# rishabhgoel0213/ZeroClone

Hardware: AMD Instinct MI355X
Metric: MCTS node-expansions/sec (whole node), Connect4 800 sims/move at 1/2/4/8 MI355X (higher is better)
Workload: dtype f64

## Files before the change

zeroclone_amd/csrc/c4_search.hip:

```cpp
#include "c4_device.h"
#include "counter_rng.h"

namespace zc {
namespace {


__device__ __forceinline__ uint64_t readlane64(uint64_t x, int l) {
    return ((uint64_t)(uint32_t)__builtin_amdgcn_readlane((int)(x >> 32), l) << 32) |
           (uint64_t)(uint32_t)__builtin_amdgcn_readlane((int)x, l);
}

__device__ __forceinline__ uint32_t mbcnt(uint64_t m) {
    return __builtin_amdgcn_mbcnt_hi((uint32_t)(m >> 32), __builtin_amdgcn_mbcnt_lo((uint32_t)m, 0u));
}

__device__ __forceinline__ uint32_t scan_add32(uint32_t x) {
    x += (uint32_t)__builtin_amdgcn_update_dpp(0, (int)x, 0x111, 0xF, 0xF, false);
    x += (uint32_t)__builtin_amdgcn_update_dpp(0, (int)x, 0x112, 0xF, 0xF, false);
    x += (uint32_t)__builtin_amdgcn_update_dpp(0, (int)x, 0x114, 0xF, 0xF, false);
    x += (uint32_t)__builtin_amdgcn_update_dpp(0, (int)x, 0x118, 0xF, 0xF, false);
    x += (uint32_t)__builtin_amdgcn_update_dpp(0, (int)x, 0x142, 0xA, 0xF, false);
    x += (uint32_t)__builtin_amdgcn_update_dpp(0, (int)x, 0x143, 0xC, 0xF, false);
    return x;
}
// ... 4 lines not shown
    x |= (uint32_t)__builtin_amdgcn_update_dpp(0, (int)x, 0x112, 0xF, 0xF, false);
    y |= (uint32_t)__builtin_amdgcn_update_dpp(0, (int)y, 0x112, 0xF, 0xF, false);
    x |= (uint32_t)__builtin_amdgcn_update_dpp(0, (int)x, 0x114, 0xF, 0xF, false);
    y |= (uint32_t)__builtin_amdgcn_update_dpp(0, (int)y, 0x114, 0xF, 0xF, false);
    x |= (uint32_t)__builtin_amdgcn_update_dpp(0, (int)x, 0x118, 0xF, 0xF, false);
    y |= (uint32_t)__builtin_amdgcn_update_dpp(0, (int)y, 0x118, 0xF, 0xF, false);
}

__device__ __forceinline__ uint64_t in_vgpr(uint64_t x) {
    __asm__("" : "+v"(x));
    return x;
}
__device__ __forceinline__ int neg_if_le(uint32_t a, uint32_t b, int y) {
    int r;
    __asm__("s_cmp_le_u32 %1, %2\n\ts_cselect_b32 %0, -1, %3" : "=s"(r) : "s"(a), "s"(b), "s"(y) : "scc");
    return r;
}
extern "C" __device__ int zc_writelane(int x, int l, int old) __asm("llvm.amdgcn.writelane.i32");
__device__ __forceinline__ uint32_t ff1(uint64_t m) {
    uint32_t r;
    __asm__("s_ff1_i32_b64 %0, %1" : "=s"(r) : "s"(m));
    return r;
}

#ifndef ZC_RV
#define ZC_RV 0
#endif
__device__ __forceinline__ void set_prio(int lvl) {
    if (lvl >= 3) __builtin_amdgcn_s_setprio(3);
    else if (lvl == 2) __builtin_amdgcn_s_setprio(2);
    else if (lvl == 1) __builtin_amdgcn_s_setprio(1);
    else __builtin_amdgcn_s_setprio(0);
}
#if defined(ZC_DIAG_WASTE) || defined(ZC_DIAG_UCT)
#define ZC_ROLLOUT_COUNTS 0
#else
#define ZC_ROLLOUT_COUNTS 1
#endif
#ifndef ZC_RSTAMP
#define ZC_RSTAMP 0
#endif
#define RMARK(k)                                                    \
    do {                                                            \
        if (ZC_RSTAMP && sub) {                                     \
            __builtin_amdgcn_sched_barrier(0);                      \
            const uint64_t now_ = __builtin_amdgcn_s_memtime();     \
            __builtin_amdgcn_sched_barrier(0);                      \
            if (ZC_RSTAMP == (k)) *sub += now_ - t_;                \
            t_ = now_;                                              \
        }                                                           \
    } while (0)
template <class R>
__device__ void c4_rollouts(Leaf *L, int nb, R &rng, const uint32_t *s_order, Counters &cn,
                            uint64_t *sub = nullptr) {
    uint64_t t_ = ZC_RSTAMP && sub ? __builtin_amdgcn_s_memtime() : 0;
    const uint32_t lane = lane_id();
    const uint32_t lrow = lane >> 4;
    constexpr uint32_t kTop3 = ViewBits<R>::kBits - 3u;
    const uint32_t *const s_dorder = draw_order_table(s_order);
    const uint64_t second_rows = __ballot((lrow & 1u) != 0);
    const uint32_t d1 = lrow < 2 ? 1u : 6u, d2 = lrow < 2 ? 7u : 8u;
    const uint32_t pairbits = lane < 49u ? (1u << (lane / 7u)) | (1u << (lane % 7u)) : 0u;
    __builtin_amdgcn_s_waitcnt(0x0F70);
    for (int g = 0; g < nb; g += 64) {
      uint32_t lm_v = 0, ow_v = 0, hp_v = 0;
      int room_v = 0;
      int val_v = 0, q_v = 0;
      {
        const int jj = g + (int)lane;
        if (jj < nb) {
            lm_v = L[jj].meta;
            ow_v = s_dorder[lm_v >> 25];
            const uint64_t x0 = L[jj].p0, x1 = L[jj].p1;
            const uint64_t op_v = (lm_v >> 24) & 1u ? x0 : x1;
            room_v = has_four(op_v) ? -2 : 41 - __popcll(x0 | x1);
            const uint64_t oc = x0 | x1;
            for (int c = 0; c < 7; ++c) hp_v |= (uint32_t)__popcll((oc >> (7 * c)) & 0x3Full) << (4 * c);
#if ZC_ROLLOUT_COUNTS
            cn.blocks += room_v >= 0 ? 1 : 0;
#endif
        }
      }
      const int jend = min(nb, g + 64);
      for (int j = g; j < jend; ++j) {
        RMARK(6);
        const int jl = j - g;
        const uint32_t lm = (uint32_t)__builtin_amdgcn_readlane((int)lm_v, jl);
        uint4 pw;
        __builtin_memcpy(&pw, &L[j], sizeof pw);
        uint64_t x0 = ((uint64_t)pw.y << 32) | pw.x, x1 = ((uint64_t)pw.w << 32) | pw.z;
        uint64_t S1 = (lm >> 24) & 1u ? ~second_rows : second_rows;
        uint32_t hp = (uint32_t)__builtin_amdgcn_readlane((int)hp_v, jl);
        const uint32_t low0 = (uint32_t)__builtin_amdgcn_readlane((int)ow_v, jl);
        const int room0 = __builtin_amdgcn_readlane(room_v, jl);
        int val = (room0 + 1) >> 1;
        int q = 0;
        RMARK(1);
        if (room0 >= 0) {
            int room = room0;
            int mask = (int)(lm >> 25);
            uint32_t ow = low0;
            uint32_t thr = (ow >> 24) & 15u;
            uint32_t owp = s_dorder[(uint32_t)mask & ~pairbits];
            uint32_t ew, l0, lf, endlane, endply, col, sc;
            uint64_t F, mine;
            auto block = [&]() __attribute__((always_inline)) {
                RMARK(6);
                uint32_t wv;
                uint64_t A;
                rng_need(rng);
                wv = rng_view(rng) >> kTop3;
                A = __ballot(wv < thr);
                if (__builtin_expect(A == 0ull, 0)) {
                    do {
                        rng_eat(rng, (uint32_t)kWin);
                        rng_need(rng);
                        wv = rng_view(rng) >> kTop3;
                        A = __ballot(wv < thr);
                    } while (A == 0ull);
                }
                RMARK(2);
                const uint32_t cap_r = min((uint32_t)room, 30u);
                uint32_t qk = mbcnt(A);
                col = (ow >> (3 * wv)) & 7u;
                uint32_t one = mask_sel0(A, 1u << (4 * col));
                sc = scan_add32(one);
                uint32_t row = ((sc - one + hp) >> (4 * col)) & 15u;
                uint32_t nacc = (uint32_t)__popcll(A);
                F = __ballot(row == 5u);
                uint64_t E0 = A & (F | __ballot(qk >= min(cap_r, nacc - 1u)));
                l0 = (uint32_t)__builtin_ctzll(E0);
                const uint64_t G = A & F & __ballot(qk < cap_r);
                lf = ff1(G);
#ifdef ZC_DIAG_WASTE
                const uint32_t l0f = l0;
#endif
                RMARK(3);
                if (lf == l0) {
                    const uint32_t cf = (uint32_t)__builtin_amdgcn_readlane((int)col, (int)lf);
                    const uint32_t ow2 = (uint32_t)__builtin_amdgcn_readlane((int)owp, (int)(8u * cf));
                    const uint32_t thr2 = (ow2 >> 24) & 15u;
                    const uint64_t high = ~1ull << lf;
                    A = (A & ~high) | (__ballot(wv < thr2) & high);
                    qk = mbcnt(A);
                    col = mask_sel(high, col, (ow2 >> (3 * wv)) & 7u);
                    one = mask_sel0(A, 1u << (4 * col));
                    sc = scan_add32(one);
                    row = ((sc - one + hp) >> (4 * col)) & 15u;
                    nacc = (uint32_t)__popcll(A);
                    F = __ballot(row == 5u) & high;
                    E0 = A & (F | __ballot(qk >= min(cap_r, nacc - 1u)));
                    l0 = (uint32_t)__builtin_ctzll(E0);
                }
                RMARK(4);
                const uint32_t c = ((qk & 1u) << 4) | ((qk >> 1) & 15u) | (qk & 32u);
                const uint32_t b = __umul24(col, 7u) + row;
                const uint32_t pl = (uint32_t)__builtin_amdgcn_ds_permute((int)(mask_sel(A, 63u, c) << 2), (int)b);
                const uint32_t pb = __builtin_amdgcn_permlane32_swap(pl, pl, false, false)[0];
                const uint64_t bit = 1ull << (pb & 63u);
                uint32_t blo = (uint32_t)bit, bhi = (uint32_t)(bit >> 32);
                scan_or16x2(blo, bhi);
                mine = ((uint64_t)bhi << 32) | blo;
                x0 = in_vgpr(x0);
                x1 = in_vgpr(x1);
                const uint64_t bd = (((uint64_t)mask_sel(S1, (uint32_t)(x0 >> 32), (uint32_t)(x1 >> 32)) << 32) |
                                     mask_sel(S1, (uint32_t)x0, (uint32_t)x1)) | mine;
                const uint64_t m1 = bd & (bd >> d1), m2 = bd & (bd >> d2);
                const uint64_t f4 = (m1 & (m1 >> (2 * d1))) | (m2 & (m2 >> (2 * d2)));
                const uint64_t W = __ballot(f4 != 0ull);
                const uint32_t W32 = (uint32_t)W | (uint32_t)(W >> 32);
                const uint64_t Ew = A & __ballot(((W32 >> (c & 31u)) & 1u) != 0u);
                ew = ff1(Ew);
                endlane = min(ew, l0);
                endply = (uint32_t)__builtin_amdgcn_readlane((int)qk, (int)endlane);
                rng_eat(rng, endlane + 1u);
#ifdef ZC_DIAG_WASTE
                cn.add(cn.blocks, lf == l0f && endlane < lf ? 1 : 0);
                cn.add(cn.plies, lf == l0f ? 1 : 0);
#endif
                room -= (int)endply + 1;
                RMARK(5);
// ... 68 lines not shown
                    const uint32_t h = (uint32_t)__popcll(((me | op) >> (7u * col)) & 0x3Full);
                    me |= 1ull << (7u * col + h);
                    ++q;
                    ++stones;
                    if (h == 5u) legal &= ~(1u << col);
                    if (has_four(me)) {
                        val = (q & 1) ? 1 : -1;
                        break;
                    }
                    if (stones == 42) {
                        val = 0;
                        break;
                    }
                    const uint64_t t = me;
                    me = op;
                    op = t;
                }
            }
            L[j].val = val;
        }
        int tot = q;
        for (int o = 32; o > 0; o >>= 1) tot += __shfl_xor(tot, o);
        cn.add(cn.plies, tot);
    }
}


__constant__ const uint64_t kEvery[8] = {0ull,
                                         0xFFFFFFFFFFFFFFFFull,
                                         0x5555555555555555ull,
                                         0x9249249249249249ull,
                                         0x1111111111111111ull,
                                         0x1084210842108421ull,
                                         0x1041041041041041ull,
                                         0x8102040810204081ull};

__device__ __forceinline__ uint64_t lanes_in(int lo, int hi) {
    const uint64_t below_hi = hi >= 64 ? ~0ull : (1ull << hi) - 1ull;
    return below_hi & ~((1ull << lo) - 1ull);
}


__device__ __forceinline__ float max8(float v) {
    float m;
    __asm__("s_nop 1\n\t"
            "v_max_f32_dpp %0, %1, %1 quad_perm:[1,0,3,2] row_mask:0xf bank_mask:0xf\n\t"
            "s_nop 1\n\t"
            "v_max_f32_dpp %0, %0, %0 quad_perm:[2,3,0,1] row_mask:0xf bank_mask:0xf\n\t"
            "s_nop 1\n\t"
            "v_max_f32_dpp %0, %0, %0 row_half_mirror row_mask:0xf bank_mask:0xf"
            : "=&v"(m)
            : "v"(v));
    return m;
}
__device__ __forceinline__ int uct_select8(uint64_t vmask, int32_t na, int32_t wa, double lg, double c, float cf,
                                           float delta, int *how = nullptr) {
    const float r = __builtin_amdgcn_rcpf((float)na);
    const float s = __builtin_amdgcn_sqrtf((float)lg * r);
    const float S = __builtin_fmaf(cf, s, (float)wa * r);
    const float Sv = __uint_as_float(mask_sel(vmask, 0xFF800000u, __float_as_uint(S)));
    const float thr = max8(Sv) - delta;
    const uint64_t C = vmask & ~__ballot(Sv < thr);
    const int first = __builtin_ctzll(C);
    if (how) *how = 0;
    if ((C & (C - 1ull)) == 0ull) return first;
    const int32_t na0 = __builtin_amdgcn_readlane(na, first), wa0 = __builtin_amdgcn_readlane(wa, first);
    if (how) *how = 1;
    if ((C & ~__ballot(((na ^ na0) | (wa ^ wa0)) == 0)) == 0ull) return first;
    if (how) *how = 2;
    const bool valid = (vmask >> (lane_id() & 7u)) & 1ull;
    const double q = valid ? (double)wa / (double)na : 0.0;
    const double v = valid ? fma(c, sqrt(lg / (double)na), q) : -INFINITY;
    int bi;
    max8_first(v, &bi);
    return bi;
}

__device__ __forceinline__ WalkEnd walk_hbm_prefetch(const Tree &t, ConstDouble *logtab, uint64_t rp0, uint64_t rp1,
                                                     int rturn, int done, double c, float delta, Counters &cn,
                                                     int &status) {
    const uint32_t lane = lane_id();
    const uint32_t k = lane & 7u, cs = lane >> 3;
    const float cf = (float)c;
    (void)cn;
    int node = 0, depth = 0, turn = rturn, nN = done;
    uint64_t b0 = rp0, b1 = rp1;
    uint32_t pathv = (lane == 0) ? 0x00FF0000u : 0u;
    const uint8_t *R0 = t.rec(0);
    uint32_t u = uni(((const uint32_t *)R0)[1]), ow = uni(((const uint32_t *)R0)[3]);
    uint32_t ch = ((const uint16_t *)(R0 + 16))[k];
    int32_t na = ((const int32_t *)(R0 + 32))[k];
    int32_t wa = ((const int32_t *)(R0 + 64))[k];
    for (;;) {
        if (untried_count(u)) break;
        if (depth >= kMaxDepth - 2) {
            status = ZC_STATUS_INTERNAL;
            u = 0;
            break;
        }
        const uint32_t nm = u >> 28;
        const uint32_t cid = (uint32_t)__builtin_amdgcn_ds_bpermute((int)(cs << 2), (int)ch);
        uint32_t pch = 0xFFFFu, phd = 0u;
        int32_t pna = 0, pwa = 0;
        if (cs < nm && cid != 0xFFFFu) {
            const uint8_t *Rc = t.rec((int)cid);
            phd = ((const uint32_t *)Rc)[lane & 3u];
            pch = ((const uint16_t *)(Rc + 16))[k];
            pna = ((const int32_t *)(Rc + 32))[k];
            pwa = ((const int32_t *)(Rc + 64))[k];
        }
        const double lg = logtab[nN];
        int best;
        const uint64_t vmask = ((1ull << nm) - 1ull) & __ballot(ch != 0xFFFF) & 0xFFull;
        const uint64_t unvisited = vmask & __ballot(na == 0);
        if (vmask == 0ull) break;
        if (unvisited) {
            best = __builtin_ctzll(unvisited);
        } else {
#ifdef ZC_DIAG_UCT
            int how;
            best = uct_select8(vmask, na, wa, lg, c, cf, delta, &how);
            cn.add(cn.plies, how != 0);
            cn.add(cn.blocks, how == 2);
#else
            best = uct_select8(vmask, na, wa, lg, c, cf, delta);
#endif
        }
        nN = __builtin_amdgcn_readlane(na, best);
        const uint64_t bit = drop_bit(b0 | b1, (int)((ow >> (3 * best)) & 7u));
        if (turn) b1 |= bit; else b0 |= bit;
        turn ^= 1;
        node = __builtin_amdgcn_readlane((int)ch, best);
        ++depth;
        if (lane == (uint32_t)depth) pathv = (uint32_t)node | ((uint32_t)best << 16);
        const int src = (int)((8u * (uint32_t)best + k) << 2);
        ch = (uint32_t)__builtin_amdgcn_ds_bpermute(src, (int)pch);
        na = __builtin_amdgcn_ds_bpermute(src, pna);
        wa = __builtin_amdgcn_ds_bpermute(src, pwa);
        u = (uint32_t)__builtin_amdgcn_readlane((int)phd, 8 * best + 1);
        ow = (uint32_t)__builtin_amdgcn_readlane((int)phd, 8 * best + 3);
    }
    return WalkEnd{node, depth, turn, b0, b1, pathv, u, ow, ch};
}

__device__ __forceinline__ uint32_t draw_class_bfe(uint32_t cnt) {
    return (6u << 16) | (((0xE480u >> (2u * cnt)) & 3u) << 3);
}

__device__ __forceinline__ uint32_t draw_table(uint32_t w3) {
    const uint32_t lane = lane_id();
    const uint32_t t3 = lane < 62u ? w3 : 7u;
    uint32_t nx = 0;
#pragma unroll
    for (uint32_t c = 0; c < 4; ++c) {
        const uint64_t s = __ballot(t3 < 4u + c) >> lane;
        const uint32_t f = s ? lane + 1u + (uint32_t)__builtin_ctzll(s) : 63u;
        nx |= f << (8u * c);
    }
    return nx;
}

__device__ __forceinline__ void write_lane(int &v, uint32_t x, int i) {
    __asm__("v_writelane_b32 %0, %1, m0" : "+v"(v) : "s"(x), "{m0}"(i));
}

__device__ __forceinline__ uint32_t draw_step(uint32_t nx, uint32_t q, uint32_t op) {
// ... 201 lines not shown
        const uint32_t c_lmask = (e_cd & 0x7Fu) & ~(filled ? 1u << col : 0u);
        uint32_t c_low = e_ow;
        if (act && filled) c_low = s_order[c_lmask];
        if (act) {
            *(uint4 *)&fresh[lane] = make_uint4(untried_init((c_low >> 24) & 15u), c_low,
                                                (uint32_t)parent | (mi << 16) | (ldepth << 24), c_lmask);
            leaves[lane] = Leaf{tn ? e_p0 : (e_p0 | bit), tn ? (e_p1 | bit) : e_p1,
                                ((uint32_t)f0 + lane) | (ldepth << 16) | ((tn ^ 1u) << 24) | (c_lmask << 25), 0,
                                c_low, 0};
        }
    }
    if (T >= 0) {
        const uint64_t tp0 = ((uint64_t)(uint32_t)__builtin_amdgcn_readlane(v_b0h, T) << 32) |
                             (uint32_t)__builtin_amdgcn_readlane(v_b0l, T);
        const uint64_t tp1 = ((uint64_t)(uint32_t)__builtin_amdgcn_readlane(v_b1h, T) << 32) |
                             (uint32_t)__builtin_amdgcn_readlane(v_b1l, T);
        const uint32_t tcm = (uint32_t)__builtin_amdgcn_readlane(v_cd, T) & 0x7Fu;
        const uint32_t tow = (uint32_t)__builtin_amdgcn_readlane(v_ow, T);
        const uint32_t meta = (uint32_t)(f0 + 63 - __clzll(Z | 1ull)) | (((uint32_t)we.depth + (uint32_t)T) << 16) |
                              (((uint32_t)we.turn ^ ((uint32_t)T & 1u)) << 24) | (tcm << 25);
        for (int jj = D + (int)lane; jj < nb; jj += 64) leaves[jj] = Leaf{tp0, tp1, meta, 0, tow, 0};
    }
    wave_mem_order();
    if (act && seg != 0) {
        Fresh &P = fresh[parent - f0];
        P.ch[mi] = (uint16_t)(f0 + (int)lane);
        atomicAnd(&P.u, ~(1u << mi));
    }
    uint32_t slotbit = (act && seg == 0) ? 1u << mi : 0u;
    slotbit |= (uint32_t)dpp<0xB1>((int)slotbit);
    slotbit |= (uint32_t)dpp<0x4E>((int)slotbit);
    slotbit |= (uint32_t)dpp<0x141>((int)slotbit);
    const uint32_t ucl = uni(slotbit);
    const uint32_t sent =
        (uint32_t)__builtin_amdgcn_ds_permute((int)(((act && seg == 0) ? mi : 63u) << 2), (int)((uint32_t)f0 + lane));
    fs.x_ch = ((ucl >> (lane & 7u)) & 1u) ? sent : we.ch;
    fs.x_u = we.u & ~ucl;
    fs.x0_dirty = true;
    fs.planned = true;
    fs.D = D;
    fs.Sm = Sm;
    fs.Z = Z;
    nnodes = f0 + D;
    wave_mem_order();
    {
        const uint32_t dep = act ? (uint32_t)we.depth + seg + 1u : 0u;
        int dsum = 0;
#pragma unroll
        for (int bit = 0; bit < 6; ++bit) dsum += __popcll(__ballot((dep >> bit) & 1u)) << bit;
        cn.add(cn.expansions, D);
        cn.add(cn.depth_sum, dsum);
    }
    stamp.mark(3);
}

constexpr int kSearchWaves = 4;
__host__ __device__ constexpr size_t kWaveSpare(int bs) { return 32 * ((size_t)bs + 1); }
__host__ __device__ constexpr size_t c4_search_wave_lds(int bs) {
    return ((size_t)kLRingBytes + (size_t)kLDrawBytes + (sizeof(Leaf) + sizeof(Fresh)) * (size_t)bs +
            kWaveSpare(bs) + 15) & ~(size_t)15;
}
static_assert(c4_search_wave_lds(32) == 8800 && c4_search_wave_lds(32) <= 9536, "per-wave LDS at batch 32");
static_assert(4 * (kTabBytes + kSearchWaves * c4_search_wave_lds(32)) <= 160 * 1024, "four workgroups per CU");

struct SearchLds {
    uint32_t *s_order;
    uint32_t *ring;
    Fresh *fresh;
    Leaf *leaves;
};

__device__ __forceinline__ SearchLds search_lds(uint8_t *s_dyn, int bs) {
    const uint32_t wave = threadIdx.x >> 6;
    uint8_t *const s_wave = s_dyn + kTabBytes + (size_t)wave * c4_search_wave_lds(bs);
    SearchLds L;
    L.s_order = (uint32_t *)s_dyn;
    L.ring = (uint32_t *)s_wave;
    constexpr size_t kRings = (size_t)kLRingBytes + (size_t)kLDrawBytes;
    L.fresh = (Fresh *)(s_wave + kRings);
    L.leaves = (Leaf *)(s_wave + kRings + sizeof(Fresh) * (size_t)bs);
    return L;
}

template <bool STAMP, bool PHILOX, int WALK = 0>
__device__ __forceinline__ void search_move(const SearchParams &p, const SearchLds &L, int gl, int g, const Tree &t,
                                            LRng &rng, uint32_t tag, Counters &cn, int &status, int &done_io,
                                            int &nnodes_io, const int32_t *stop = nullptr, int32_t budget = 0,
                                            int *lagp = nullptr, const int32_t *progress = nullptr, int mv = 0) {
    int lag = lagp ? *lagp : 0;
    const uint32_t lane = lane_id();
    const uint32_t *const s_order = L.s_order;
    Fresh *const fresh = L.fresh;
    Leaf *const leaves = L.leaves;
    ConstDouble *logtab = (ConstDouble *)p.a.logtab;
    if (done_io == 0) {
        const zc_c4_state root = p.roots[gl];
        node_init(t, 0, 0xFFFF, 0xFF, 0, uni(s_order[legal_mask(uni64(root.stones[0]) | uni64(root.stones[1]))]));
    }
    int nnodes = done_io == 0 ? 1 : nnodes_io;
    wave_mem_order();

    Stamp<STAMP> stamp;
    int done = done_io;
    while (done < p.sims) {
        const int nb = min(p.bs, p.sims - done);
        stamp.mark(0);

        FlushSel fs;
        {
            const zc_c4_state root = p.roots[gl];
            if (p.bs < 64)
                select_flush_plan<STAMP>(t, fresh, leaves, s_order, logtab, rng, cn, stamp, nnodes, status,
                                         uni64(root.stones[0]), uni64(root.stones[1]), uni(root.turn), done, nb,
                                         p.c, p.uct_delta, fs);
            else
                select_flush<false, STAMP>(t, fresh, leaves, nullptr, s_order, logtab, rng, cn, stamp, nnodes,
                                           status, uni64(root.stones[0]), uni64(root.stones[1]), uni(root.turn),
                                           done, nb, p.c, fs);
        }
        const int f0 = fs.f0, d0 = fs.d0;

        const size_t wlog = (size_t)g * p.sims + done;
        const size_t wfl = (size_t)g * ((p.sims + p.bs - 1) / p.bs) + done / p.bs;
        if (WALK == 2) {
            for (int jj = (int)lane; jj < nb; jj += kBlock) leaves[jj].val = p.walk_vals[wlog + jj];
            lrng_skip(rng, uni(p.walk_words[wfl]));
        } else if (PHILOX) {
            c4_rollouts_philox(leaves, nb, sel_table(s_order),
                               make_uint2((uint32_t)p.philox_seed, (uint32_t)(p.philox_seed >> 32)), (uint32_t)done,
                               tag, (uint32_t)g, cn);
        } else {
            const int32_t u0 = rng.use();
            constexpr int kRolloutPrio = 1;
            set_prio(lag + kRolloutPrio);
            c4_rollouts(leaves, nb, rng, s_order, cn, STAMP ? &stamp.ph[7] : nullptr);
            set_prio(lag);
            if (WALK == 1) {
                wave_mem_order();
                for (int jj = (int)lane; jj < nb; jj += kBlock) p.walk_vals[wlog + jj] = (int8_t)leaves[jj].val;
                if (lane == 0) p.walk_words[wfl] = (uint32_t)(rng.use() - u0);
            }
        }
        wave_mem_order();
        stamp.mark(4);

        const bool pre = lane >= 1 && lane <= (uint32_t)d0;
        const int par = __shfl((int)(fs.ppath & 0xFFFFu), (int)lane - 1);
        const int act = (int)(fs.ppath >> 16);
        int32_t na0 = 0, w0 = 0, spent_v = 0;
        if (stop) spent_v = __hip_atomic_load(stop, __ATOMIC_RELAXED, __HIP_MEMORY_SCOPE_AGENT);
        if (progress)
            spent_v = __hip_atomic_load(progress, __ATOMIC_RELAXED, __HIP_MEMORY_SCOPE_AGENT);
        if (pre) {
            na0 = t.na(par)[act];
            w0 = t.w(par)[act];
        }
        const int32_t spent = stop || progress ? uni(spent_v) : 0;
        if (fs.planned) {
            const int jj = (int)lane;
            int v = 0, dl = 0;
            if (jj < nb) {
                v = leaves[jj].val;
                dl = (int)((leaves[jj].meta >> 16) & 0xFFu);
            }
            const int sv = (dl & 1) ? -v : v;
            const int P = (int)scan_add32((uint32_t)sv);
            const int S = __builtin_amdgcn_readlane(P, 63);
            const int suf = S - P + sv;
            const uint64_t above = jj < 63 ? fs.Sm >> (jj + 1) : 0ull;
            const int nxt = above ? jj + 1 + __builtin_ctzll(above) : fs.D;
            const int sufn = __builtin_amdgcn_ds_bpermute(nxt << 2, suf);
            const bool isz = (fs.Z >> jj) & 1ull;
            const int na_e = 1 + (isz ? nb - nxt : 0);
            const int ss = sv + (isz ? sufn : 0);
            const int w_e = (dl & 1) ? ss : -ss;
            if (pre) {
                const int dw = (lane & 1u) ? S : -S;
                t.na(par)[act] = na0 + nb;
                t.w(par)[act] = w0 + dw;
            }
            stamp.mark(5);
            if (jj < fs.D) {
                const Fresh &F = fresh[jj];
                const uint4 ch = *(const uint4 *)F.ch;
                const uint32_t link = F.link;
                uint8_t *R = t.rec(f0 + jj);
                *(uint4 *)R = make_uint4(0u, F.u, link, F.ow);
                *(uint4 *)(R + 16) = ch;
                const int pn = (int)(link & 0xFFFFu);
                if (pn >= f0) {
                    const int pa = (int)((link >> 16) & 0xFFu);
                    t.na(pn)[pa] = na_e;
                    t.w(pn)[pa] = w_e;
                }
            }
            if (fs.x0_dirty) {
                const int x0node = fs.x0node;
                const uint32_t x_ch = fs.x_ch;
                const bool xf = x_ch != 0xFFFF && (int)x_ch >= f0;
                const int src = (xf ? (int)x_ch - f0 : 0) << 2;
                const int xna = __builtin_amdgcn_ds_bpermute(src, na_e);
                const int xw = __builtin_amdgcn_ds_bpermute(src, w_e);
                if (lane == 0) t.hdr(x0node)[1] = fs.x_u;
                if (lane < kSlots) {
                    t.child(x0node)[lane] = (uint16_t)x_ch;
                    if (xf) {
                        t.na(x0node)[lane] = xna;
                        t.w(x0node)[lane] = xw;
                    }
                }
            }
        } else {
            int S = 0;
            for (int base = 0; base < nb; base += 64) {
                const int jj = base + (int)lane;
                int v = 0, d = -1, sv = 0;
                if (jj < nb) {
                    const uint32_t meta = leaves[jj].meta;
                    v = leaves[jj].val;
                    d = (int)((meta >> 16) & 0xFFu);
                    sv = (d & 1) ? -v : v;
                }
                S += __popcll(__ballot(sv > 0)) - __popcll(__ballot(sv < 0));
                int nd = jj < nb ? (int)(leaves[jj].meta & 0xFFFFu) : -1, l = d;
                while (__ballot(nd >= f0)) {
                    if (nd >= f0) {
                        const int fi = nd - f0;
                        const int vl = ((d - l) & 1) ? -v : v;
                        atomicAdd(&fresh[fi].na, 1);
                        atomicAdd(&fresh[fi].w, -vl);
                        nd = (int)(fresh[fi].link & 0xFFFFu);
                        --l;
                    }
                }
            }
            if (pre) {
                const int dw = (lane & 1u) ? S : -S;
                t.na(par)[act] = na0 + nb;
                t.w(par)[act] = w0 + dw;
            }
            wave_mem_order();
            stamp.mark(5);

            if (fs.x0_dirty) {
                const int x0node = fs.x0node;
                const uint32_t x_ch = fs.x_ch;
                if (lane == 0) t.hdr(x0node)[1] = fs.x_u;
                if (lane < kSlots) {
                    t.child(x0node)[lane] = (uint16_t)x_ch;
                    if (x_ch != 0xFFFF && (int)x_ch >= f0) {
                        t.na(x0node)[lane] = fresh[x_ch - f0].na;
                        t.w(x0node)[lane] = fresh[x_ch - f0].w;
                    }
                }
            }
            {
                const int nf = nnodes - f0;
                for (int base = 0; base < nf * 8; base += 64) {
                    const int idx = base + (int)lane;
                    if (idx < nf * 8) {
                        const int r = idx >> 3, slot = idx & 7;
                        const Fresh &F = fresh[r];
                        const uint16_t c = F.ch[slot];
                        int32_t na = 0, w = 0;
                        if (c != 0xFFFF) {
                            na = fresh[c - f0].na;
                            w = fresh[c - f0].w;
                        }
                        uint8_t *R = t.rec(f0 + r);
                        if (slot == 0) *(uint4 *)R = make_uint4(0u, F.u, F.link, F.ow);
                        ((uint16_t *)(R + 16))[slot] = c;
                        ((int32_t *)(R + 32))[slot] = na;
                        ((int32_t *)(R + 64))[slot] = w;
                    }
                }
            }
        }
        wave_mem_order();
        stamp.mark(6);
        done += nb;
        if (stop && done < p.sims && status == 0 && uni(spent) >= budget) break;
        if (progress) {
            const int64_t own = ((int64_t)mv * p.sims + done) * p.n_games, avg = (int64_t)spent * p.sims;
            const int64_t mvn = (int64_t)p.sims * p.n_games;
            lag = own >= avg ? 0 : own + mvn <= avg ? 2 : 1;
            set_prio(lag);
        }
    }
    done_io = done;
    nnodes_io = nnodes;
    if (lagp) *lagp = lag;
    if (STAMP && lane == 0)
        for (int k_ = 0; k_ < kPhases; ++k_) p.a.phase[kPhases * (size_t)g + k_] += (int64_t)stamp.ph[k_];
}

__device__ __forceinline__ int best_column(const Tree &t, int &na_col) {
    const uint32_t lane = lane_id();
    const uint32_t k = lane & 7u;
    const uint32_t u = uni(t.hdr(0)[1]);
    const uint32_t ow = uni(t.hdr(0)[3]);
    const uint32_t nm = u >> 28;
    int bv = (k < nm) ? t.na(0)[k] : -1;
    int bi = (int)k;
    argmax8(bv, bi);
    const int best = uni(bi);
    int pos = -1;
    for (uint32_t s = 0; s < nm; ++s)
        if (((ow >> (3 * s)) & 7u) == lane) pos = (int)s;
    na_col = pos >= 0 ? t.na(0)[pos] : 0;
    return (int)((ow >> (3 * best)) & 7u);
}

template <bool STAMP, bool PHILOX, int WALK>
__device__ __forceinline__ void search_games(const SearchParams &p, uint8_t *s_dyn) {
    const SearchLds L = search_lds(s_dyn, p.bs);
    load_tables(L.s_order);
    __syncthreads();

    const uint32_t lane = lane_id();
    const int gl = (int)(blockIdx.x * (blockDim.x >> 6) + (threadIdx.x >> 6));
    if (gl >= p.n_games) return;
    const int g = p.game_ids ? uni(p.game_ids[gl]) : p.first_game + gl;
    {
        const zc_c4_state root = p.roots[gl];
        const uint64_t rp0 = uni64(root.stones[0]), rp1 = uni64(root.stones[1]);
        const int rturn = uni(root.turn);
        if (!valid_state(rp0, rp1, rturn) || legal_mask(rp0 | rp1) == 0) {
            if (lane == 0) {
                zc_game_stats st{};
                st.status = valid_state(rp0, rp1, rturn) ? ZC_STATUS_NO_MOVES : ZC_STATUS_BAD_STATE;
                p.out_stats[gl] = st;
                p.out_move[gl] = -1;
            }
            if (lane < 7) p.out_na[(size_t)gl * 7 + lane] = 0;
            return;
        }
    }
    const Arena &a = p.a;
    const Tree t{a.nodes + (size_t)g * p.M * kRecBytes};
    LRng rng;
    const uint64_t use0 = uni64(a.rngpos[2 * (size_t)g]);
    lrng_open(rng, L.ring, a.ring + (size_t)g * kRingWords, use0, uni64(a.rngpos[2 * (size_t)g + 1]));
    Counters cn;
    int status = 0, done = 0, nnodes = 1;
    search_move<STAMP, PHILOX, WALK>(p, L, gl, g, t, rng, uni((uint32_t)use0), cn, status, done, nnodes);
    int na_col;
    const int col = best_column(t, na_col);
    if (lane < 7) p.out_na[(size_t)gl * 7 + lane] = na_col;
    const int32_t plies = Counters::total(cn.plies), blocks = Counters::total(cn.blocks);
    if (lane == 0) {
        p.out_move[gl] = col;
        zc_game_stats st{};
        st.status = status;
        st.expansions = cn.expansions;
        st.depth_sum = cn.depth_sum;
        st.leaves = p.sims;
        st.rollout_plies = plies;
        st.rollout_blocks = blocks;
        st.rng_words = rng.use();
        p.out_stats[gl] = st;
    }
    lrng_close(rng, a.ring + (size_t)g * kRingWords, use0, a.rngpos + 2 * (size_t)g);
}

template <bool STAMP, bool PHILOX>
__global__ __launch_bounds__(kSearchWaves * kBlock, 4) void c4_search_kernel(SearchParams p) {
    extern __shared__ __attribute__((aligned(16))) uint8_t s_dyn[];
    search_games<STAMP, PHILOX, 0>(p, s_dyn);
}

template <int WALK>
__global__ __launch_bounds__(kSearchWaves * kBlock, 4) void c4_walk_kernel(SearchParams p) {
    extern __shared__ __attribute__((aligned(16))) uint8_t s_dyn[];
    search_games<false, false, WALK>(p, s_dyn);
}

template <bool PHILOX>
__global__ __launch_bounds__(kSearchWaves * kBlock, 4) void c4_selfplay_kernel(SearchParams p) {
    extern __shared__ __attribute__((aligned(16))) uint8_t s_dyn[];
    const SearchLds L = search_lds(s_dyn, p.bs);
    load_tables(L.s_order);
    __syncthreads();

    const uint32_t lane = lane_id();
    const int gl = (int)(blockIdx.x * (blockDim.x >> 6) + (threadIdx.x >> 6));
    if (gl >= p.n_games) return;
    const int g = p.first_game + gl;
    const Arena &a = p.a;
    const Tree t{a.nodes + (size_t)g * p.M * kRecBytes};
    LRng rng;
    const uint64_t use0 = uni64(a.rngpos[2 * (size_t)g]);
    lrng_open(rng, L.ring, a.ring + (size_t)g * kRingWords, use0, uni64(a.rngpos[2 * (size_t)g + 1]));
    Counters cn;
    int status = 0;
    int finished = 0;
    int mv = 0;
    int64_t leaves = 0;
    uint64_t t_start = 0, t_last = 0;
    if (p.tstamps) t_start = t_last = __builtin_amdgcn_s_memrealtime();
    int lag = 0;
    uint4 cy = a.carry[g];
    cy = make_uint4(uni(cy.x), uni(cy.y), uni(cy.z), 0u);
    bool resume = cy.x != 0;
    for (; mv < p.moves; ++mv) {
        if (p.ticket && !resume) {
            int tk = 0;
            if (lane == 0) tk = atomicAdd(p.ticket, 1);
            if (uni(tk) >= p.budget) break;
        }
        if (p.tstamps) t_last = __builtin_amdgcn_s_memrealtime();
        zc_c4_state root = p.roots[gl];
        uint64_t s0 = uni64(root.stones[0]), s1 = uni64(root.stones[1]);
        int turn = uni(root.turn);
        if (!valid_state(s0, s1, turn) || legal_mask(s0 | s1) == 0) {
            status = ZC_STATUS_BAD_STATE;
            break;
        }
        int done = resume ? (int)cy.x : 0, nnodes = resume ? (int)cy.y : 1;
        const uint32_t tag = resume ? cy.z : uni((uint32_t)(use0 + (uint64_t)(int64_t)rng.use()));
        const int done0 = done;
        search_move<false, PHILOX>(p, L, gl, g, t, rng, tag, cn, status, done, nnodes, p.carry ? p.ticket : nullptr,
                                   p.budget, &lag, p.progress, mv);
        if (p.progress && lane == 0) atomicAdd(p.progress, 1);
        leaves += done - done0;
        if (done < p.sims) {
            if (lane == 0) a.carry[g] = make_uint4((uint32_t)done, (uint32_t)nnodes, tag, 0u);
            break;
        }
        if (resume && lane == 0) a.carry[g] = make_uint4(0u, 0u, 0u, 0u);
        resume = false;
        int na_col;
        const int col = best_column(t, na_col);
        const uint64_t bit = drop_bit(s0 | s1, col);
        if (turn) s1 |= bit; else s0 |= bit;
        const bool won = has_four(turn ? s1 : s0);
        turn ^= 1;
        const int r = won ? turn * 2 - 1 : ((s0 | s1) == kFull ? 0 : ZC_C4_ONGOING);
        const size_t o = (size_t)mv * p.n_games + gl;
        if (p.out_na && lane < 7) p.out_na[o * 7 + lane] = na_col;
        if (lane == 0) {
            zc_c4_state post;
            post.stones[0] = s0;
            post.stones[1] = s1;
            post.turn = turn;
            post.reserved = 0;
            p.out_states[o] = post;
            p.out_moves16[o] = (int16_t)col;
            p.out_results[o] = r;
            p.io_roots[gl] = r == ZC_C4_ONGOING ? post : zc_c4_state{{0, 0}, 0, 0};
        }
        finished += r != ZC_C4_ONGOING;
        wave_mem_order();
    }
    if (p.ticket && lane == 0) atomicMax(p.ticket + 1, mv);
    if (p.tstamps && lane == 0) {
        uint64_t *ts = p.tstamps + 4 * (size_t)g;
        ts[0] = t_start;
        ts[1] = t_last;
        ts[2] = __builtin_amdgcn_s_memrealtime();
        const uint32_t hw = (uint32_t)__builtin_amdgcn_s_getreg(4 | (15 << 11)) |
                            ((uint32_t)__builtin_amdgcn_s_getreg(20 | (3 << 11)) << 16);
        ts[3] = (uint64_t)mv | ((uint64_t)hw << 32);
    }
    for (int k = mv + (int)lane; k < p.moves; k += kBlock) {
        const size_t o = (size_t)k * p.n_games + gl;
        p.out_moves16[o] = -1;
        p.out_results[o] = ZC_SLOT_SKIP;
    }
    const int32_t plies = Counters::total(cn.plies), blocks = Counters::total(cn.blocks);
    if (lane == 0) {
        zc_game_stats st{};
        st.status = status;
        st.expansions = cn.expansions;
        st.depth_sum = cn.depth_sum;
        st.leaves = leaves;
        st.rollout_plies = plies;
        st.rollout_blocks = blocks;
        st.rng_words = rng.use();
        st.reserved = finished;
        p.out_stats[gl] = st;
    }
    lrng_close(rng, a.ring + (size_t)g * kRingWords, use0, a.rngpos + 2 * (size_t)g);
}

__global__ __launch_bounds__(kBlock) void c4_rollout_debug_kernel(Arena a, int first_game, int n,
                                                                  const zc_c4_state *states, int32_t *out_value,
                                                                  int64_t *out_words) {
    __shared__ Leaf s_leaf[1];
    __shared__ uint32_t s_order[kTabBytes / 4];
    load_tables(s_order);
    __syncthreads();
    const uint32_t lane = lane_id();
    const int gl = blockIdx.x;
    if (gl >= n) return;
    const int g = first_game + gl;
    Rng rng;
    const uint64_t use0 = uni64(a.rngpos[2 * (size_t)g]);
    rng_open(rng, a.ring + (size_t)g * kRingWords, use0, uni64(a.rngpos[2 * (size_t)g + 1]));
    const zc_c4_state s = states[gl];
    if (lane == 0) {
        s_leaf[0].p0 = s.stones[0];
        s_leaf[0].p1 = s.stones[1];
        s_leaf[0].meta = ((uint32_t)s.turn << 24) | ((uint32_t)legal_mask(s.stones[0] | s.stones[1]) << 25);
        s_leaf[0].ow = s_order[legal_mask(s.stones[0] | s.stones[1])];
    }
    wave_mem_order();
    Counters cn;
    c4_rollouts(s_leaf, 1, rng, s_order, cn);
    wave_mem_order();
    if (lane == 0) {
        out_value[gl] = s_leaf[0].val;
        out_words[gl] = rng.use();
        rng_close(rng, use0, a.rngpos + 2 * (size_t)g);
    }
}

__global__ __launch_bounds__(kBlock) void c4_rollout_seq_kernel(Arena a, int g, int n, const zc_c4_state *states,
                                                                int32_t *out_value, int64_t *out_words) {
    __shared__ Leaf s_leaf[kBlock];
    __shared__ uint32_t s_order[kTabBytes / 4];
    load_tables(s_order);
    __syncthreads();
    const uint32_t lane = lane_id();
    Rng rng;
    const uint64_t use0 = uni64(a.rngpos[2 * (size_t)g]);
    rng_open(rng, a.ring + (size_t)g * kRingWords, use0, uni64(a.rngpos[2 * (size_t)g + 1]));
    Counters cn;
    for (int base = 0; base < n; base += kBlock) {
        const int cnt = min(kBlock, n - base);
        if ((int)lane < cnt) {
            const zc_c4_state s = states[base + lane];
            s_leaf[lane].p0 = s.stones[0];
            s_leaf[lane].p1 = s.stones[1];
            s_leaf[lane].meta = ((uint32_t)s.turn << 24) | ((uint32_t)legal_mask(s.stones[0] | s.stones[1]) << 25);
            s_leaf[lane].ow = s_order[legal_mask(s.stones[0] | s.stones[1])];
        }
        wave_mem_order();
        rng_fill(rng, rng.use() + kLookahead);
        c4_rollouts(s_leaf, cnt, rng, s_order, cn);
        wave_mem_order();
        if ((int)lane < cnt) out_value[base + lane] = s_leaf[lane].val;
        wave_mem_order();
    }
    if (lane == 0) {
        out_words[0] = rng.use();
        rng_close(rng, use0, a.rngpos + 2 * (size_t)g);
    }
}

__global__ void c4_play_kernel(int n, zc_c4_state *states, const int32_t *moves, int32_t *results, int reset) {
    const int i = blockIdx.x * blockDim.x + threadIdx.x;
    if (i >= n) return;
    const int col = moves[i];
    if (col < 0 || col > 6) {
        results[i] = ZC_C4_ONGOING;
        return;
    }
    zc_c4_state s = states[i];
    const int turn = s.turn & 1;
    s.stones[turn] |= drop_bit(s.stones[0] | s.stones[1], col);
    s.turn = turn ^ 1;
    int r = ZC_C4_ONGOING;
    if (has_four(s.stones[turn])) r = s.turn * 2 - 1;
    else if ((s.stones[0] | s.stones[1]) == kFull) r = 0;
    if (reset && r != ZC_C4_ONGOING) s = zc_c4_state{{0, 0}, 0, 0};
    states[i] = s;
    results[i] = r;
}

__global__ void uct_debug_kernel(int n, const double *logn, const int32_t *na, const double *q, double c,
                                 double *out) {
    const int i = blockIdx.x * blockDim.x + threadIdx.x;
    if (i >= n) return;
    out[i] = na[i] == 0 ? INFINITY : fma(c, sqrt(logn[i] / (double)na[i]), q[i]);
}

__global__ __launch_bounds__(kBlock) void c4_uct_select_debug_kernel(int n, const uint16_t *ch, const int32_t *na,
                                                                     const int32_t *wa, const int32_t *bigN,
                                                                     const double *logtab, double c, float delta,
                                                                     int32_t *out_slot, int32_t *out_how) {
    const uint32_t lane = lane_id();
    const uint32_t k = lane & 7u;
    const float cf = (float)c;
    for (int i = (int)blockIdx.x; i < n; i += (int)gridDim.x) {
        const uint32_t chk = ch[8 * (size_t)i + k];
        const int32_t nak = na[8 * (size_t)i + k], wak = wa[8 * (size_t)i + k];
        const double lg = ((ConstDouble *)logtab)[uni(bigN[i])];
        const uint64_t vmask = __ballot(chk != 0xFFFF) & 0xFFull;
        const uint64_t unvisited = vmask & __ballot(nak == 0);
        int best = -1, how = 0;
        if (vmask != 0ull) {
            if (unvisited) best = __builtin_ctzll(unvisited);
            else best = uct_select8(vmask, nak, wak, lg, c, cf, delta, &how);
        }
        if (lane == 0) {
            out_slot[i] = best;
            out_how[i] = how;
        }
    }
}

}

static_assert(kTabBytes + kSearchWaves * c4_search_wave_lds(314) <= 160 * 1024, "batch 314: the last with four waves");
static_assert(kTabBytes + kSearchWaves * c4_search_wave_lds(315) > 160 * 1024, "batch 315: the first with two waves");
static_assert(kTabBytes + 2 * c4_search_wave_lds(512) <= 160 * 1024, "batch 512 (max_batch) fits two waves");
static int c4_search_wpg(int bs) {
    int w = kSearchWaves;
    while (w > 1 && kTabBytes + (size_t)w * c4_search_wave_lds(bs) > (size_t)(160 * 1024)) w >>= 1;
    return w;
}

size_t c4_search_lds_bytes(int bs) { return kTabBytes + (size_t)c4_search_wpg(bs) * c4_search_wave_lds(bs); }

void launch_c4_search(const SearchParams &p, hipStream_t s) {
    const int wpg = c4_search_wpg(p.bs);
    const size_t lds = c4_search_lds_bytes(p.bs);
    const dim3 grid((p.n_games + wpg - 1) / wpg), block(wpg * kBlock);
    if (p.philox) {
        if (p.stamp)
            hipLaunchKernelGGL((c4_search_kernel<true, true>), grid, block, lds, s, p);
        else
            hipLaunchKernelGGL((c4_search_kernel<false, true>), grid, block, lds, s, p);
    } else {
        if (p.stamp)
            hipLaunchKernelGGL((c4_search_kernel<true, false>), grid, block, lds, s, p);
        else
            hipLaunchKernelGGL((c4_search_kernel<false, false>), grid, block, lds, s, p);
    }
}

void launch_c4_walk(const SearchParams &p, int mode, hipStream_t s) {
    const int wpg = c4_search_wpg(p.bs);
    const size_t lds = c4_search_lds_bytes(p.bs);
    const dim3 grid((p.n_games + wpg - 1) / wpg), block(wpg * kBlock);
    if (mode == 1)
        hipLaunchKernelGGL((c4_walk_kernel<1>), grid, block, lds, s, p);
    else
        hipLaunchKernelGGL((c4_walk_kernel<2>), grid, block, lds, s, p);
}

void launch_c4_selfplay(const SearchParams &p, hipStream_t s) {
    const int wpg = c4_search_wpg(p.bs);
    const size_t lds = c4_search_lds_bytes(p.bs);
    const dim3 grid((p.n_games + wpg - 1) / wpg), block(wpg * kBlock);
    if (p.philox)
        hipLaunchKernelGGL((c4_selfplay_kernel<true>), grid, block, lds, s, p);
    else
        hipLaunchKernelGGL((c4_selfplay_kernel<false>), grid, block, lds, s, p);
}

int c4_selfplay_resident_games(int bs, int philox, int *out) {
    const int wpg = c4_search_wpg(bs);
    int blocks = 0, dev = 0, cus = 0;
    const void *fn = philox ? (const void *)c4_selfplay_kernel<true> : (const void *)c4_selfplay_kernel<false>;
    if (hipOccupancyMaxActiveBlocksPerMultiprocessor(&blocks, fn, wpg * kBlock, c4_search_lds_bytes(bs)) != hipSuccess)
        return -1;
    if (hipGetDevice(&dev) != hipSuccess) return -1;
    if (hipDeviceGetAttribute(&cus, hipDeviceAttributeMultiprocessorCount, dev) != hipSuccess) return -1;
    *out = blocks * cus * wpg;
    return 0;
}

void launch_c4_rollout_debug(const Arena &a, int M, int first_game, int n, const zc_c4_state *states,
                             int32_t *out_value, int64_t *out_words, hipStream_t s) {
    (void)M;
    hipLaunchKernelGGL(c4_rollout_debug_kernel, dim3(n), dim3(kBlock), 0, s, a, first_game, n, states, out_value,
                       out_words);
}

void launch_c4_rollout_seq(const Arena &a, int game, int n, const zc_c4_state *states, int32_t *out_value,
                           int64_t *out_words, hipStream_t s) {
    hipLaunchKernelGGL(c4_rollout_seq_kernel, dim3(1), dim3(kBlock), 0, s, a, game, n, states, out_value, out_words);
}

void launch_c4_play(int n, zc_c4_state *states, const int32_t *moves, int32_t *results, int reset, hipStream_t s) {
    hipLaunchKernelGGL(c4_play_kernel, dim3((n + 255) / 256), dim3(256), 0, s, n, states, moves, results, reset);
}

void launch_uct_debug(int n, const double *logn, const int32_t *na, const double *q, double c, double *out,
                      hipStream_t s) {
    hipLaunchKernelGGL(uct_debug_kernel, dim3((n + 255) / 256), dim3(256), 0, s, n, logn, na, q, c, out);
}

void launch_c4_uct_select_debug(int n, const uint16_t *ch, const int32_t *na, const int32_t *wa, const int32_t *bigN,
                                const double *logtab, double c, float delta, int32_t *out_slot, int32_t *out_how,
                                hipStream_t s) {
    hipLaunchKernelGGL(c4_uct_select_debug_kernel, dim3(n < 8192 ? n : 8192), dim3(kBlock), 0, s, n, ch, na, wa, bigN,
                       logtab, c, delta, out_slot, out_how);
}

}
```

Before: 3.689 billion.

## Specialize search kernels on mode and planning, skip dead rollout leaves

The rollout loop now iterates only over lanes whose leaf is live, found with a ballot and find-first-set, instead of walking every leaf and branching on terminal ones. Terminal leaf values are precomputed per lane. The search and selfplay kernels gain compile-time MODE and PLANNED template parameters, so runtime checks on stop, progress, ticket and bs disappear and each variant compiles only its own path. Asm barriers pin the walk's constants to scalar or vector registers. The cost is more kernel instantiations and larger code size, and occupancy queries now take the minimum across modes.

```diff
diff --git a/zeroclone_amd/csrc/c4_search.hip b/zeroclone_amd/csrc/c4_search.hip
--- a/zeroclone_amd/csrc/c4_search.hip
+++ b/zeroclone_amd/csrc/c4_search.hip
@@ -110,9 +110,12 @@
         }
       }
       const int jend = min(nb, g + 64);
-      for (int j = g; j < jend; ++j) {
+      val_v = room_v < 0 ? (room_v + 1) >> 1 : 0;
+      uint64_t live = __ballot(g + (int)lane < nb && room_v >= 0);
+      while (live) {
         RMARK(6);
-        const int jl = j - g;
+        const int jl = (int)ff1(live), j = g + jl;
+        __asm__("s_bitset0_b64 %0, %1" : "+s"(live) : "s"(jl));
         const uint32_t lm = (uint32_t)__builtin_amdgcn_readlane((int)lm_v, jl);
         uint4 pw;
         __builtin_memcpy(&pw, &L[j], sizeof pw);
@@ -121,10 +124,9 @@
         uint32_t hp = (uint32_t)__builtin_amdgcn_readlane((int)hp_v, jl);
         const uint32_t low0 = (uint32_t)__builtin_amdgcn_readlane((int)ow_v, jl);
         const int room0 = __builtin_amdgcn_readlane(room_v, jl);
-        int val = (room0 + 1) >> 1;
-        int q = 0;
+        int val, q;
         RMARK(1);
-        if (room0 >= 0) {
+        {
             int room = room0;
             int mask = (int)(lm >> 25);
             uint32_t ow = low0;
@@ -359,6 +361,13 @@
     const uint32_t lane = lane_id();
     const uint32_t k = lane & 7u, cs = lane >> 3;
     const float cf = (float)c;
+    __asm__("" : "+v"(delta));
+    __asm__ volatile("" : "+s"(logtab));
+    {
+        uint64_t cb = (uint64_t)__double_as_longlong(c);
+        __asm__ volatile("" : "+s"(cb));
+        c = __longlong_as_double((long long)cb);
+    }
     (void)cn;
     int node = 0, depth = 0, turn = rturn, nN = done;
     uint64_t b0 = rp0, b1 = rp1;
@@ -726,12 +735,18 @@
     return L;
 }
 
-template <bool STAMP, bool PHILOX, int WALK = 0>
+enum : int {
+    kModePlain = 0,
+    kModePaced = 1,
+    kModePooled = 2,
+    kModeCarry = 3,
+};
+template <bool STAMP, bool PHILOX, int WALK, int MODE, bool PLANNED>
 __device__ __forceinline__ void search_move(const SearchParams &p, const SearchLds &L, int gl, int g, const Tree &t,
                                             LRng &rng, uint32_t tag, Counters &cn, int &status, int &done_io,
-                                            int &nnodes_io, const int32_t *stop = nullptr, int32_t budget = 0,
-                                            int *lagp = nullptr, const int32_t *progress = nullptr, int mv = 0) {
-    int lag = lagp ? *lagp : 0;
+                                            int &nnodes_io, int *lagp = nullptr, int mv = 0) {
+    constexpr bool kPaced = MODE == kModePaced, kCarry = MODE == kModeCarry;
+    int lag = kPaced ? *lagp : 0;
     const uint32_t lane = lane_id();
     const uint32_t *const s_order = L.s_order;
     Fresh *const fresh = L.fresh;
@@ -753,7 +768,7 @@
         FlushSel fs;
         {
             const zc_c4_state root = p.roots[gl];
-            if (p.bs < 64)
+            if constexpr (PLANNED)
                 select_flush_plan<STAMP>(t, fresh, leaves, s_order, logtab, rng, cn, stamp, nnodes, status,
                                          uni64(root.stones[0]), uni64(root.stones[1]), uni(root.turn), done, nb,
                                          p.c, p.uct_delta, fs);
@@ -776,9 +791,11 @@
         } else {
             const int32_t u0 = rng.use();
             constexpr int kRolloutPrio = 1;
-            set_prio(lag + kRolloutPrio);
+            if constexpr (kPaced) set_prio(lag + kRolloutPrio);
+            else __builtin_amdgcn_s_setprio(kRolloutPrio);
             c4_rollouts(leaves, nb, rng, s_order, cn, STAMP ? &stamp.ph[7] : nullptr);
-            set_prio(lag);
+            if constexpr (kPaced) set_prio(lag);
+            else __builtin_amdgcn_s_setprio(0);
             if (WALK == 1) {
                 wave_mem_order();
                 for (int jj = (int)lane; jj < nb; jj += kBlock) p.walk_vals[wlog + jj] = (int8_t)leaves[jj].val;
@@ -792,15 +809,14 @@
         const int par = __shfl((int)(fs.ppath & 0xFFFFu), (int)lane - 1);
         const int act = (int)(fs.ppath >> 16);
         int32_t na0 = 0, w0 = 0, spent_v = 0;
-        if (stop) spent_v = __hip_atomic_load(stop, __ATOMIC_RELAXED, __HIP_MEMORY_SCOPE_AGENT);
-        if (progress)
-            spent_v = __hip_atomic_load(progress, __ATOMIC_RELAXED, __HIP_MEMORY_SCOPE_AGENT);
+        if constexpr (kCarry) spent_v = __hip_atomic_load(p.ticket, __ATOMIC_RELAXED, __HIP_MEMORY_SCOPE_AGENT);
+        if constexpr (kPaced) spent_v = __hip_atomic_load(p.progress, __ATOMIC_RELAXED, __HIP_MEMORY_SCOPE_AGENT);
         if (pre) {
             na0 = t.na(par)[act];
             w0 = t.w(par)[act];
         }
-        const int32_t spent = stop || progress ? uni(spent_v) : 0;
-        if (fs.planned) {
+        const int32_t spent = kCarry || kPaced ? uni(spent_v) : 0;
+        if constexpr (PLANNED) {
             const int jj = (int)lane;
             int v = 0, dl = 0;
             if (jj < nb) {
@@ -923,8 +939,9 @@
         wave_mem_order();
         stamp.mark(6);
         done += nb;
-        if (stop && done < p.sims && status == 0 && uni(spent) >= budget) break;
-        if (progress) {
+        if constexpr (kCarry)
+            if (done < p.sims && status == 0 && uni(spent) >= p.budget) break;
+        if constexpr (kPaced) {
             const int64_t own = ((int64_t)mv * p.sims + done) * p.n_games, avg = (int64_t)spent * p.sims;
             const int64_t mvn = (int64_t)p.sims * p.n_games;
             lag = own >= avg ? 0 : own + mvn <= avg ? 2 : 1;
@@ -933,7 +950,7 @@
     }
     done_io = done;
     nnodes_io = nnodes;
-    if (lagp) *lagp = lag;
+    if constexpr (kPaced) *lagp = lag;
     if (STAMP && lane == 0)
         for (int k_ = 0; k_ < kPhases; ++k_) p.a.phase[kPhases * (size_t)g + k_] += (int64_t)stamp.ph[k_];
 }
@@ -955,7 +972,7 @@
     return (int)((ow >> (3 * best)) & 7u);
 }
 
-template <bool STAMP, bool PHILOX, int WALK>
+template <bool STAMP, bool PHILOX, int WALK, bool PLANNED>
 __device__ __forceinline__ void search_games(const SearchParams &p, uint8_t *s_dyn) {
     const SearchLds L = search_lds(s_dyn, p.bs);
     load_tables(L.s_order);
@@ -987,7 +1004,8 @@
     lrng_open(rng, L.ring, a.ring + (size_t)g * kRingWords, use0, uni64(a.rngpos[2 * (size_t)g + 1]));
     Counters cn;
     int status = 0, done = 0, nnodes = 1;
-    search_move<STAMP, PHILOX, WALK>(p, L, gl, g, t, rng, uni((uint32_t)use0), cn, status, done, nnodes);
+    search_move<STAMP, PHILOX, WALK, kModePlain, PLANNED>(p, L, gl, g, t, rng, uni((uint32_t)use0), cn, status, done,
+                                                          nnodes);
     int na_col;
     const int col = best_column(t, na_col);
     if (lane < 7) p.out_na[(size_t)gl * 7 + lane] = na_col;
@@ -1007,20 +1025,21 @@
     lrng_close(rng, a.ring + (size_t)g * kRingWords, use0, a.rngpos + 2 * (size_t)g);
 }
 
-template <bool STAMP, bool PHILOX>
+template <bool STAMP, bool PHILOX, bool PLANNED>
 __global__ __launch_bounds__(kSearchWaves * kBlock, 4) void c4_search_kernel(SearchParams p) {
     extern __shared__ __attribute__((aligned(16))) uint8_t s_dyn[];
-    search_games<STAMP, PHILOX, 0>(p, s_dyn);
-}
-
-template <int WALK>
+    search_games<STAMP, PHILOX, 0, PLANNED>(p, s_dyn);
+}
+
+template <int WALK, bool PLANNED>
 __global__ __launch_bounds__(kSearchWaves * kBlock, 4) void c4_walk_kernel(SearchParams p) {
     extern __shared__ __attribute__((aligned(16))) uint8_t s_dyn[];
-    search_games<false, false, WALK>(p, s_dyn);
-}
-
-template <bool PHILOX>
+    search_games<false, false, WALK, PLANNED>(p, s_dyn);
+}
+
+template <bool PHILOX, int MODE, bool PLANNED>
 __global__ __launch_bounds__(kSearchWaves * kBlock, 4) void c4_selfplay_kernel(SearchParams p) {
+    constexpr bool kTickets = MODE == kModePooled || MODE == kModeCarry;
     extern __shared__ __attribute__((aligned(16))) uint8_t s_dyn[];
     const SearchLds L = search_lds(s_dyn, p.bs);
     load_tables(L.s_order);
@@ -1047,7 +1066,7 @@
     cy = make_uint4(uni(cy.x), uni(cy.y), uni(cy.z), 0u);
     bool resume = cy.x != 0;
     for (; mv < p.moves; ++mv) {
-        if (p.ticket && !resume) {
+        if (kTickets && !resume) {
             int tk = 0;
             if (lane == 0) tk = atomicAdd(p.ticket, 1);
             if (uni(tk) >= p.budget) break;
@@ -1063,11 +1082,10 @@
         int done = resume ? (int)cy.x : 0, nnodes = resume ? (int)cy.y : 1;
         const uint32_t tag = resume ? cy.z : uni((uint32_t)(use0 + (uint64_t)(int64_t)rng.use()));
         const int done0 = done;
-        search_move<false, PHILOX>(p, L, gl, g, t, rng, tag, cn, status, done, nnodes, p.carry ? p.ticket : nullptr,
-                                   p.budget, &lag, p.progress, mv);
-        if (p.progress && lane == 0) atomicAdd(p.progress, 1);
+        search_move<false, PHILOX, 0, MODE, PLANNED>(p, L, gl, g, t, rng, tag, cn, status, done, nnodes, &lag, mv);
+        if (MODE == kModePaced && lane == 0) atomicAdd(p.progress, 1);
         leaves += done - done0;
-        if (done < p.sims) {
+        if (MODE == kModeCarry && done < p.sims) {
             if (lane == 0) a.carry[g] = make_uint4((uint32_t)done, (uint32_t)nnodes, tag, 0u);
             break;
         }
@@ -1096,7 +1114,7 @@
         finished += r != ZC_C4_ONGOING;
         wave_mem_order();
     }
-    if (p.ticket && lane == 0) atomicMax(p.ticket + 1, mv);
+    if (kTickets && lane == 0) atomicMax(p.ticket + 1, mv);
     if (p.tstamps && lane == 0) {
         uint64_t *ts = p.tstamps + 4 * (size_t)g;
         ts[0] = t_start;
@@ -1257,49 +1275,63 @@
 
 size_t c4_search_lds_bytes(int bs) { return kTabBytes + (size_t)c4_search_wpg(bs) * c4_search_wave_lds(bs); }
 
+using SearchKernel = void (*)(SearchParams);
+template <bool STAMP, bool PHILOX>
+static SearchKernel c4_search_instance(int bs) {
+    return bs < 64 ? c4_search_kernel<STAMP, PHILOX, true> : c4_search_kernel<STAMP, PHILOX, false>;
+}
+template <bool PHILOX, int MODE>
+static SearchKernel c4_selfplay_mode(int bs) {
+    return bs < 64 ? c4_selfplay_kernel<PHILOX, MODE, true> : c4_selfplay_kernel<PHILOX, MODE, false>;
+}
+static int c4_selfplay_mode_of(const SearchParams &p) {
+    return !p.ticket ? kModePaced : p.carry ? kModeCarry : kModePooled;
+}
+static SearchKernel c4_selfplay_instance(int bs, int philox, int mode) {
+    if (philox)
+        return mode == kModePaced    ? c4_selfplay_mode<true, kModePaced>(bs)
+               : mode == kModeCarry ? c4_selfplay_mode<true, kModeCarry>(bs)
+                                    : c4_selfplay_mode<true, kModePooled>(bs);
+    return mode == kModePaced    ? c4_selfplay_mode<false, kModePaced>(bs)
+           : mode == kModeCarry ? c4_selfplay_mode<false, kModeCarry>(bs)
+                                : c4_selfplay_mode<false, kModePooled>(bs);
+}
+
 void launch_c4_search(const SearchParams &p, hipStream_t s) {
     const int wpg = c4_search_wpg(p.bs);
     const size_t lds = c4_search_lds_bytes(p.bs);
     const dim3 grid((p.n_games + wpg - 1) / wpg), block(wpg * kBlock);
-    if (p.philox) {
-        if (p.stamp)
-            hipLaunchKernelGGL((c4_search_kernel<true, true>), grid, block, lds, s, p);
-        else
-            hipLaunchKernelGGL((c4_search_kernel<false, true>), grid, block, lds, s, p);
-    } else {
-        if (p.stamp)
-            hipLaunchKernelGGL((c4_search_kernel<true, false>), grid, block, lds, s, p);
-        else
-            hipLaunchKernelGGL((c4_search_kernel<false, false>), grid, block, lds, s, p);
-    }
+    const SearchKernel k = p.philox ? (p.stamp ? c4_search_instance<true, true>(p.bs) : c4_search_instance<false, true>(p.bs))
+                                    : (p.stamp ? c4_search_instance<true, false>(p.bs) : c4_search_instance<false, false>(p.bs));
+    hipLaunchKernelGGL(k, grid, block, lds, s, p);
 }
 
 void launch_c4_walk(const SearchParams &p, int mode, hipStream_t s) {
     const int wpg = c4_search_wpg(p.bs);
     const size_t lds = c4_search_lds_bytes(p.bs);
     const dim3 grid((p.n_games + wpg - 1) / wpg), block(wpg * kBlock);
-    if (mode == 1)
-        hipLaunchKernelGGL((c4_walk_kernel<1>), grid, block, lds, s, p);
-    else
-        hipLaunchKernelGGL((c4_walk_kernel<2>), grid, block, lds, s, p);
+    const SearchKernel k = mode == 1 ? (p.bs < 64 ? c4_walk_kernel<1, true> : c4_walk_kernel<1, false>)
+                                     : (p.bs < 64 ? c4_walk_kernel<2, true> : c4_walk_kernel<2, false>);
+    hipLaunchKernelGGL(k, grid, block, lds, s, p);
 }
 
 void launch_c4_selfplay(const SearchParams &p, hipStream_t s) {
     const int wpg = c4_search_wpg(p.bs);
     const size_t lds = c4_search_lds_bytes(p.bs);
     const dim3 grid((p.n_games + wpg - 1) / wpg), block(wpg * kBlock);
-    if (p.philox)
-        hipLaunchKernelGGL((c4_selfplay_kernel<true>), grid, block, lds, s, p);
-    else
-        hipLaunchKernelGGL((c4_selfplay_kernel<false>), grid, block, lds, s, p);
+    hipLaunchKernelGGL(c4_selfplay_instance(p.bs, p.philox, c4_selfplay_mode_of(p)), grid, block, lds, s, p);
 }
 
 int c4_selfplay_resident_games(int bs, int philox, int *out) {
     const int wpg = c4_search_wpg(bs);
     int blocks = 0, dev = 0, cus = 0;
-    const void *fn = philox ? (const void *)c4_selfplay_kernel<true> : (const void *)c4_selfplay_kernel<false>;
-    if (hipOccupancyMaxActiveBlocksPerMultiprocessor(&blocks, fn, wpg * kBlock, c4_search_lds_bytes(bs)) != hipSuccess)
-        return -1;
+    for (const int mode : {kModePooled, kModeCarry}) {
+        int b = 0;
+        const void *fn = (const void *)c4_selfplay_instance(bs, philox, mode);
+        if (hipOccupancyMaxActiveBlocksPerMultiprocessor(&b, fn, wpg * kBlock, c4_search_lds_bytes(bs)) != hipSuccess)
+            return -1;
+        blocks = mode == kModePooled || b < blocks ? b : blocks;
+    }
     if (hipGetDevice(&dev) != hipSuccess) return -1;
     if (hipDeviceGetAttribute(&cus, hipDeviceAttributeMultiprocessorCount, dev) != hipSuccess) return -1;
     *out = blocks * cus * wpg;
```

After: 3.730 billion, median of 6. 1.01x the previous value.
